# ZongyueQin/SessionSimilaritySearch

Measured on AMD Instinct MI355X. Metric: session queries/sec, higher is better.
Workload: dtype f32

## Files before the change

sessionsimilaritysearch_amd/csrc/ip_topk.hip:

```cpp
#include "scan.h"

namespace sss {

namespace {
constexpr int PROF_RING = 512;
struct Prof {
    bool on = false;
    int n = 0;
    hipEvent_t ev[2 * PROF_RING];
    bool made = false;
};
Prof g_prof[MAX_DEVICES];
}

extern "C" int sss_profile_enable(int on) {
    Prof& p = g_prof[current_device()];
    if (on && !p.made) {
        for (int i = 0; i < 2 * PROF_RING; ++i)
            if (hipEventCreate(&p.ev[i]) != hipSuccess) { set_error("profile_enable: hipEventCreate failed"); return SSS_EHIP; }
        p.made = true;
    }
    p.on = on != 0;
    p.n = 0;
    return SSS_OK;
// ... 12 lines not shown
    *launches = p.n;
    p.n = 0;
    return SSS_OK;
}

static bool fused_shape_ok(int d, int dtype) {
    const int rb = d * elem_bytes(dtype);
    return format_of(dtype) && (rb == 256 || rb == 512 || rb == 1024);
}

int check_scan_source(const char* what, int exact_dtype, int scan_dtype, int d, bool long_rows, const void* c_scan, int corpus_shift,
                      float corpus_resid, long n, long nq) {
    if (long_rows && exact_dtype == DT_I8) {
        set_error("%s: int8 rows (dtype %d) have no long-row scan: d in {256,512,1024} on the fused scan, else the exhaustive kernels", what, DT_I8);
        return SSS_EINVAL;
    }
    if (!(long_rows ? long_shape_ok(d, exact_dtype, scan_dtype) : scan_pair_ok(exact_dtype, scan_dtype, false) && fused_shape_ok(d, scan_dtype))) {
        set_error("%s: no scan of type %d for dtype %d, d %d", what, scan_dtype, exact_dtype, d);
        return SSS_EINVAL;
    }
    if (!c_scan || (reinterpret_cast<uintptr_t>(c_scan) & 15)) {
        set_error("%s: scan image (the %s) missing or not 16-byte aligned", what, format_of(scan_dtype)->name);
        return SSS_EINVAL;
    }
    if (scan_dtype == DT_F16 && (corpus_shift < -160 || corpus_shift > 160 || !(corpus_resid >= 0.f))) {
        set_error("%s: corpus_shift %d outside [-160, 160] or corpus_resid_norm %g not >= 0", what, corpus_shift, (double)corpus_resid);
        return SSS_EINVAL;
    }
    if (n >= (1L << 31) - 1024 || nq >= (1L << 31)) { set_error("%s: n and nq must be < 2^31", what); return SSS_EINVAL; }
    return SSS_OK;
}

ThrArgs thr_args(const void* q, const void* c_exact, int exact_dtype, int scan_dtype, int corpus_shift, float corpus_resid,
                 float corpus_max_norm, const int* qsel, long nsel, long n, int d, int k, int cap, long id_offset) {
    ThrArgs t = {};
    t.Q = q; t.C = c_exact; t.qsel = qsel; t.nsel = (int)nsel; t.d = d; t.dtype = exact_dtype; t.k = k; t.cap = cap; t.n = n;
    t.scan_dtype = scan_dtype; t.corpus_shift = corpus_shift; t.corpus_resid = corpus_resid; t.corpus_max_norm = corpus_max_norm;
    t.id_offset = id_offset;
    return t;
}

extern "C" size_t sss_ip_topk_state_bytes(int64_t nq) { return nq > 0 ? state_words(nq) * 4 : 0; }

extern "C" size_t sss_ip_topk_workspace_bytes(int64_t nq, int64_t n, int d, int k, int dtype) {
    if (nq <= 0 || n <= 0 || k <= 0 || !corpus_dtype_ok(dtype) || !fused_shape_ok(d, dtype)) return 0;
    return make_plan(nq, n, d, k, dtype).total_bytes;
}

static size_t ip_topk_scan_workspace_bytes(long nq, long n, int d, int k, int scan_dtype) {
    if (nq <= 0 || n <= 0 || k <= 0 || !fused_shape_ok(d, scan_dtype)) return 0;
    return make_plan(nq, n, d, k, scan_dtype).total_bytes;
}

extern "C" size_t sss_ip_topk_f16_workspace_bytes(int64_t nq, int64_t n, int d, int k) {
    return ip_topk_scan_workspace_bytes(nq, n, d, k, DT_F16);
}

extern "C" int sss_f16_shift(float amax) { return f16_shift(amax); }

static int ip_topk_impl(const char* what, const void* q, long nq, const void* c_scan, int scan_dtype, int corpus_shift,
                        float corpus_resid, const void* c_exact,
                        int exact_dtype, long n, int d, int k, long id_offset, float corpus_max_norm, float* D_out, long* I_out,
                        int* status, int* unproven_count, void* state, size_t state_bytes, void* ws, size_t ws_bytes,
                        hipStream_t st, const float* bias = nullptr, int d_row = 0) {
    const bool l2 = bias != nullptr;
    if (nq <= 0 || n <= 0 || k <= 0) { set_error("%s: nq, n, k must be positive", what); return SSS_EINVAL; }
    int rc = check_scan_source(what, exact_dtype, scan_dtype, d, false, c_scan, corpus_shift, corpus_resid, n, nq);
    if (rc) return rc;
    if (k > 500) { set_error("%s: k too large (max 500)", what); return SSS_EINVAL; }
    if ((reinterpret_cast<uintptr_t>(ws) & 255) || (reinterpret_cast<uintptr_t>(state) & 15)) {
        set_error("%s: workspace must be 256-byte aligned, state 16-byte aligned", what);
        return SSS_EINVAL;
    }
    if (!state || state_bytes < sss_ip_topk_state_bytes(nq)) { set_error("%s: state %zu < %zu bytes", what, state_bytes, sss_ip_topk_state_bytes(nq)); return SSS_EWORKSPACE; }
    const ScanPlan p = make_plan(nq, n, d, k, scan_dtype);
    if (ws_bytes < p.total_bytes) { set_error("%s: workspace %zu < %zu", what, ws_bytes, p.total_bytes); return SSS_EWORKSPACE; }
    char* w = reinterpret_cast<char*>(ws);

    ScanArgs a;
    a.Q = q; a.C = c_scan; a.nq = (int)nq; a.n = (int)n;
    a.tiles_per_split = p.tiles_per_split; a.total_tiles = p.total_tiles;
    a.S = p.S; a.G = p.G; a.J = p.J; a.Ju = p.Ju; a.cert = p.cert; a.boot = p.boot; a.append = p.append; a.cap = p.cap;
    a.tau_skip = p.tau_skip;
    unsigned* sw = reinterpret_cast<unsigned*>(state);
    a.slots = sw;
    a.cnt = sw + state_off_cnt(nq);
    a.maxlast = reinterpret_cast<unsigned long long*>(sw + state_off_maxlast(nq));
    a.cand = reinterpret_cast<unsigned long long*>(w);
    a.bias = bias; a.corpus_shift = corpus_shift;
    Prof& pr = g_prof[current_device()];
    const bool prof = pr.on && pr.n < PROF_RING;
    if (prof) (void)hipEventRecord(pr.ev[2 * pr.n], st);
    rc = launch_scan(scan_dtype, d, p.tile_rows, a, st);
    if (prof) { (void)hipEventRecord(pr.ev[2 * pr.n + 1], st); ++pr.n; }
    if (rc) return rc;

    SelectArgs s;
    s.Q = q; s.C = c_exact; s.nq = (int)nq; s.d = d; s.dtype = exact_dtype; s.scan_dtype = scan_dtype; s.corpus_shift = corpus_shift; s.corpus_resid = corpus_resid;
    s.k = k; s.K2 = p.K2; s.J = p.J; s.cap = p.cap; s.tau_skip = p.tau_skip;
    s.cand = a.cand; s.slots = a.slots; s.cnt = a.cnt; s.maxlast = a.maxlast;
    s.id_offset = id_offset; s.corpus_max_norm = corpus_max_norm;
    s.D_out = D_out; s.I_out = I_out; s.status = status; s.unproven_count = unproven_count;
    s.metric = l2 ? 1 : 0;
    s.d_row = d_row;
    rc = launch_select(s, st);
    if (rc) (void)hipMemsetAsync(state, 0, sss_ip_topk_state_bytes(nq), st);
    return rc;
}

template <class Prepare, class Select>
static int run_threshold_form(const ThrArgs& t, const void* c_scan, const ScanPlan& p, Prepare prepare, Select select, hipStream_t st,
                              const float* bias = nullptr) {
    int rc = prepare();
    if (rc) return rc;
    ScanArgs a = {};
    a.Q = t.Q; a.C = c_scan; a.nq = t.nsel; a.n = (int)t.n;
    a.tiles_per_split = p.tiles_per_split; a.total_tiles = p.total_tiles;
    a.S = p.S; a.G = p.G; a.J = 0; a.Ju = 0; a.cert = 1; a.boot = 0; a.append = 0; a.cap = p.cap;
    a.slots = nullptr; a.cnt = t.cnt; a.maxlast = nullptr;
    a.cand = const_cast<unsigned long long*>(t.cand);
    a.qsel = t.qsel; a.thr = t.thr;
    a.bias = bias; a.corpus_shift = t.corpus_shift;
    rc = launch_scan(t.scan_dtype, t.d, p.tile_rows, a, st);
    if (rc) return rc;
    return select();
}

constexpr int THR_CAP = 8192;
static size_t thr_head_bytes(long nsel) { return ((size_t)nsel * 8 + 255) & ~(size_t)255; }

extern "C" size_t sss_ip_topk_threshold_workspace_bytes(int64_t nsel, int64_t n, int d, int scan) {
    if (nsel <= 0 || n <= 0 || !fused_shape_ok(d, scan)) return 0;
    return thr_head_bytes(nsel) + make_thr_plan(nsel, n, d, scan, THR_CAP).total_bytes;
}

static int topk_threshold_impl(const char* what, const void* q, const int* qsel, long nsel, const void* c_exact, int exact_dtype,
                               const void* c_scan, int scan_dtype, int corpus_shift, float corpus_resid, long n, int d, int k,
                               long id_offset, float corpus_max_norm, float* D_out, long* I_out, int* status, void* ws, size_t ws_bytes,
                               hipStream_t st, const float* bias = nullptr, int d_row = 0) {
    if (nsel <= 0 || n <= 0 || k <= 0 || !qsel) { set_error("%s: nsel, n, k must be positive", what); return SSS_EINVAL; }
    const int rc = check_scan_source(what, exact_dtype, scan_dtype, d, false, c_scan, corpus_shift, corpus_resid, n, nsel);
    if (rc) return rc;
    if (k > THR_CAP) { set_error("%s: k too large (max %d)", what, THR_CAP); return SSS_EINVAL; }
    if (reinterpret_cast<uintptr_t>(ws) & 255) { set_error("%s: workspace must be 256-byte aligned", what); return SSS_EINVAL; }
    const ScanPlan p = make_thr_plan(nsel, n, d, scan_dtype, THR_CAP);
    if (ws_bytes < thr_head_bytes(nsel) + p.total_bytes) { set_error("%s: workspace %zu < %zu", what, ws_bytes, thr_head_bytes(nsel) + p.total_bytes); return SSS_EWORKSPACE; }
    char* w = reinterpret_cast<char*>(ws);
    ThrArgs t = thr_args(q, c_exact, exact_dtype, scan_dtype, corpus_shift, corpus_resid, corpus_max_norm, qsel, nsel, n, d, k, p.cap,
                         id_offset);
    t.thr = reinterpret_cast<float*>(w);
    t.cnt = reinterpret_cast<unsigned*>(w + (size_t)nsel * 4);
    t.cand = reinterpret_cast<unsigned long long*>(w + thr_head_bytes(nsel));
    t.D_out = D_out; t.I_out = I_out; t.status = status;
    t.metric = bias != nullptr ? 1 : 0;
    t.d_row = d_row;
    return run_threshold_form(t, c_scan, p, [&] { return launch_thr_prepare(t, st); }, [&] { return launch_select_all(t, st); }, st, bias);
}

extern "C" int sss_ip_topk_threshold(const void* q, const int32_t* qsel, int64_t nsel, const void* corpus, int dtype,
                                     const void* scan_image, int scan, int corpus_shift, float corpus_resid_norm, int64_t n, int d,
                                     int k, int64_t id_offset, float corpus_max_norm, float* D_out, int64_t* I_out, int32_t* status,
                                     void* workspace, size_t workspace_bytes, void* stream) {
    hipStream_t st = static_cast<hipStream_t>(stream);
    return topk_threshold_impl("ip_topk_threshold", q, qsel, nsel, corpus, dtype, scan_image, scan, corpus_shift, corpus_resid_norm, n, d,
                               k, id_offset, corpus_max_norm, D_out, I_out, status, workspace, workspace_bytes, st);
}
// ... 185 lines not shown
```

sessionsimilaritysearch_amd/csrc/scan.h:

```cpp
#pragma once
#include "elem.h"

namespace sss {

__host__ __device__ inline int f16_shift(float amax) {
    if (!(amax > 0.f) || !(amax <= 3.4028234663852886e38f)) return 0;
    int e;
    (void)frexpf(amax, &e);
    return 13 - e;
}

constexpr int KP = 16;
constexpr int WG_QUERIES = 256;
constexpr int MAX_SLOTS = 128;
constexpr int SLOT_STRIDE = MAX_SLOTS;
constexpr unsigned ORD_NEG_INF = 0x007FFFFFu;
constexpr double ULP32_REL = 2.4e-7;
constexpr double ULP32_MIN = 1e-44;

static inline int pow2_at_least(int x) { int p = 64; while (p < x) p <<= 1; return p; }

static inline bool long_shape_ok(int d, int exact_dtype, int scan_dtype) {
    return d > 0 && d % 64 == 0 && d * elem_bytes(exact_dtype) <= 16384 && scan_pair_ok(exact_dtype, scan_dtype, true);
}

__device__ __forceinline__ double l2_chain_step(double acc, double q, double c) {
    const double dl = __dsub_rn(q, c);
    return __dadd_rn(acc, __dmul_rn(dl, dl));
}

static inline size_t state_off_cnt(long nq) { return (size_t)nq * MAX_SLOTS; }
static inline size_t state_off_maxlast(long nq) { return (state_off_cnt(nq) + (size_t)nq + 1) & ~(size_t)1; }
static inline size_t state_words(long nq) { return state_off_maxlast(nq) + 2 * (size_t)nq; }

struct ScanPlan {
    int G, S, L, K2, J, Ju, cert, boot, append, tile_rows;
    int tau_skip;
    int total_tiles, tiles_per_split, cap;
    size_t total_bytes;
};

ScanPlan make_plan(long nq, long n, int d, int k, int dtype);

struct ScanArgs {
    const void* Q;
    const void* C;
    int nq, n, tiles_per_split, total_tiles, S, G, J, Ju, cert, boot, append, cap;
    int tau_skip = 0;
    unsigned* slots;
    unsigned* cnt;
    unsigned long long* maxlast;
    unsigned long long* cand;
    const int* qsel = nullptr;
    const float* thr = nullptr;
    const float* bias = nullptr;
    int corpus_shift = 0;
};

ScanPlan make_thr_plan(long nsel, long n, int d, int scan_dtype, int cap);
int launch_scan(int dtype, int d, int tile_rows, const ScanArgs& a, hipStream_t st);
int launch_scan_l2(int dtype, int d, int tile_rows, const ScanArgs& a, hipStream_t st);

struct SelectArgs {
    const void* Q;
    const void* C;
    int nq, d, dtype, k, K2, J, cap;
    int tau_skip = 0;
    int scan_dtype;
    int corpus_shift;
    float corpus_resid;
    const unsigned long long* cand;
    unsigned* slots;
    unsigned* cnt;
    unsigned long long* maxlast;
    long id_offset;
    float corpus_max_norm;
    float* D_out;
    long* I_out;
    int* status;
    int* unproven_count;
    int metric = 0;
    int d_row = 0;
};

int launch_select(const SelectArgs& a, hipStream_t st);

struct ThrArgs {
    const void* Q;
    const void* C;
    const int* qsel;
    int nsel, d, dtype, k, cap;
    long n;
    int scan_dtype, corpus_shift;
    float corpus_resid, corpus_max_norm;
    long id_offset;
    float* thr;
    unsigned* cnt;
    const unsigned long long* cand;
    float* D_out;
    long* I_out;
    int* status;
    double* qb = nullptr;
    int qb_ready = 0;
    int keep = 0;
    int metric = 0;
    int d_row = 0;
};
int launch_thr_prepare(const ThrArgs& a, hipStream_t st);
int launch_select_all(const ThrArgs& a, hipStream_t st);
int launch_long_setup(const ThrArgs& a, int* qsel, void* qimg, float* seed, hipStream_t st);
int launch_bound_prepare(const ThrArgs& a, hipStream_t st);
int launch_range_prepare(const ThrArgs& a, const float* radius, int* qsel, hipStream_t st);
int launch_range_select(const ThrArgs& a, const float* radius, long* counts, int* status, hipStream_t st);
int launch_range_fill(const unsigned* cnt, const unsigned long long* cand, int cap, long nq, const long* lims, long id_offset, float* D,
                      long* I, hipStream_t st);

int check_scan_source(const char* what, int exact_dtype, int scan_dtype, int d, bool long_rows, const void* c_scan, int corpus_shift,
                      float corpus_resid, long n, long nq);
ThrArgs thr_args(const void* q, const void* c_exact, int exact_dtype, int scan_dtype, int corpus_shift, float corpus_resid,
                 float corpus_max_norm, const int* qsel, long nsel, long n, int d, int k, int cap, long id_offset);

size_t topk_of_scores_bytes(long nsel, long n);
int topk_of_scores(const float* scores, const int* qsel, long nsel, long n, int k, long id_offset, int metric, float* D_out,
                   long* I_out, void* tail, hipStream_t st);

}
```

sessionsimilaritysearch_amd/csrc/scan.hip:

```cpp
#include "scan_kernel.h"

namespace sss {

__device__ unsigned g_boot_expired;

extern "C" int sss_scan_boot_expired(int reset) {
    unsigned v = 0, zero = 0;
    if (hipMemcpyFromSymbol(&v, HIP_SYMBOL(g_boot_expired), sizeof(v)) != hipSuccess) { set_error("scan_boot_expired: read failed"); return SSS_EHIP; }
    if (reset && hipMemcpyToSymbol(HIP_SYMBOL(g_boot_expired), &zero, sizeof(zero)) != hipSuccess) { set_error("scan_boot_expired: reset failed"); return SSS_EHIP; }
    return (int)(v > 0x7fffffffu ? 0x7fffffffu : v);
}

int current_device() {
    int dev = 0;
    (void)hipGetDevice(&dev);
    return dev < 0 || dev >= MAX_DEVICES ? 0 : dev;
}

static int pick_splits(long n, int G, int tr) {
    int S = (256 / G) & ~7;
    if (S < 8) S = 8;
    while (S > 8 && (long)S * tr > n) S -= 8;
    return S;
}

constexpr int TR256_MIN_TILES = 24;

static size_t align256(size_t v) { return (v + 255) & ~(size_t)255; }

static ScanPlan make_plan_for(long nq, long n, int d, int k, int dtype, bool want_append);

static bool append_form_fits() {
    static int cached[MAX_DEVICES] = {};
    const int dev = current_device();
    if (cached[dev] == 0) {
        constexpr int lds = 2 * 128 * 256 + 8 * 2048;
        const void* fn = reinterpret_cast<const void*>(&k_scan<256, 128, DT_F16, 8, false, true>);
        int blocks = 0, cus = 0;
        bool ok = hipFuncSetAttribute(fn, hipFuncAttributeMaxDynamicSharedMemorySize, lds) == hipSuccess &&
                  hipOccupancyMaxActiveBlocksPerMultiprocessor(&blocks, fn, 512, lds) == hipSuccess &&
                  hipDeviceGetAttribute(&cus, hipDeviceAttributeMultiprocessorCount, dev) == hipSuccess;
        (void)hipGetLastError();
        cached[dev] = (ok && blocks >= 2 && cus >= 256) ? 1 : 2;
    }
    return cached[dev] == 1;
}

ScanPlan make_plan(long nq, long n, int d, int k, int dtype) {
    const int rb = d * elem_bytes(dtype);
    if (rb == 256 && dtype != DT_F32 && k <= KP && append_form_fits()) {
        const ScanPlan a = make_plan_for(nq, n, d, k, dtype, true);
        if (a.append) return a;
    }
    return make_plan_for(nq, n, d, k, dtype, false);
}
static ScanPlan make_plan_for(long nq, long n, int d, int k, int dtype, bool want_append) {
    ScanPlan p;
    const int rb = d * elem_bytes(dtype);
    const int wgq = rb == 1024 ? 128 : WG_QUERIES;
    p.G = (int)((nq + wgq - 1) / wgq);
    int tr = rb <= 512 ? 128 : 64;
    int S = pick_splits(n, p.G, tr);
    if (rb == 512 && (n + (long)S * 128 - 1) / ((long)S * 128) < 48) { tr = 64; S = pick_splits(n, p.G, tr); }
    if (rb == 256 && dtype != DT_F32 && n / ((long)S * 256) >= TR256_MIN_TILES) tr = 256;
    if (want_append) {
        tr = 128;
        S = pick_splits(n, p.G, tr);
        if ((long)S * p.G > 256 || (long)2 * S * tr * 7 > n) want_append = false;
        else S *= 2;
        if (!want_append) { ScanPlan none; none.append = 0; return none; }
    }
    p.tile_rows = tr;
    p.S = S;
    p.L = 2 * S;
    p.K2 = k + 2 <= KP ? (k + 2 < 8 ? 8 : k + 2) : k <= KP ? KP : k + 12;
    if ((long)p.L * KP < p.K2) p.K2 = p.L * KP;
    p.total_tiles = (int)((n + tr - 1) / tr);
    p.tiles_per_split = (p.total_tiles + S - 1) / S;
    p.cap = p.L * KP;
    const int active_splits = (p.total_tiles + p.tiles_per_split - 1) / p.tiles_per_split;
    p.J = p.K2 <= 128 ? 16 : 64;
    p.cert = 1;
    while (p.J * p.cert < p.K2 && p.cert < KP) p.cert *= 2;
    p.Ju = p.J;
    p.tau_skip = (p.cert == 1 && p.J == 16) ? 16 - p.K2 : 0;
    bool classes_ok = 2 * active_splits >= p.Ju;
    if (p.cert == 1 && p.J == 16 && active_splits < 16) {
        const int zero0 = active_splits < 8 ? 8 - active_splits : 0, zero1 = active_splits < 8 ? 8 : 16 - active_splits;
        classes_ok = zero0 <= (p.tau_skip >> 1) + (p.tau_skip & 1) && zero1 <= (p.tau_skip >> 1);
    }
    if (p.J * p.cert < p.K2 || !classes_ok) { p.J = 0; p.Ju = 0; p.tau_skip = 0; }
    p.boot = (p.J > 0 && p.cert == 1) ? 1 : 0;
    p.append = (want_append && p.boot) ? 1 : 0;
    if (want_append && !p.append) return p;
    if (p.append) p.cap = 2048;
    p.total_bytes = align256((size_t)nq * p.cap * 8);
    return p;
}

ScanPlan make_thr_plan(long nsel, long n, int d, int scan_dtype, int cap) {
    ScanPlan p = {};
    const int rb = d * elem_bytes(scan_dtype);
    const int wgq = rb == 1024 ? 128 : WG_QUERIES;
    p.G = (int)((nsel + wgq - 1) / wgq);
    p.tile_rows = rb <= 512 ? 128 : 64;
    p.S = pick_splits(n, p.G, p.tile_rows);
    p.L = 2 * p.S;
    p.total_tiles = (int)((n + p.tile_rows - 1) / p.tile_rows);
    p.tiles_per_split = (p.total_tiles + p.S - 1) / p.S;
    p.cap = cap;
    p.total_bytes = align256((size_t)nsel * cap * 8);
    return p;
}

int launch_scan(int dtype, int d, int tile_rows, const ScanArgs& a, hipStream_t st) {
    const int rb = d * elem_bytes(dtype);
    if (a.bias != nullptr) return launch_scan_l2(dtype, d, tile_rows, a, st);
    int rc = 1;
    with_dtype<true>(dtype, [&](auto dt) {
        constexpr int DT = decltype(dt)::value;
        rc = launch_shape<DT, 0>(rb, tile_rows, a, st);
    });
    if (rc != 1) return rc;
    set_error("scan: unsupported row size %d bytes", rb);
    return SSS_EINVAL;
}

}
```

sessionsimilaritysearch_amd/csrc/scan_kernel.h:

```cpp
#pragma once
#include "scan.h"
#include "scan_dev.h"

#ifndef SSS_STAGGER
#define SSS_STAGGER 1
#endif
#ifndef SSS_F32_SCHED
#define SSS_F32_SCHED 7
#endif

namespace sss {

extern __device__ unsigned g_boot_expired;

template <int RB, int TR, int DT, int NW, bool THR = false, bool AP = false, int MET = 0>
__global__ __launch_bounds__(NW * 64, AP ? 2 * (NW / 4) : NW / 4) void k_scan(const ScanArgs A) {
    constexpr int H = TR / 64;
    constexpr int CH = RB / 16;
    constexpr int NU = RB / 32;
    constexpr int TILE_BYTES = TR * RB;
    constexpr int LOADS_PER_WAVE = TR * CH / 64 / NW;
    constexpr int WGQ = NW * 32;
    constexpr bool PRECOMP = RB <= 512 && !AP;
    constexpr int TAU_LDS = 2 * TILE_BYTES;
    constexpr bool F32S = (SSS_F32_SCHED & 1) && DT == DT_F32 && !AP && !THR && RB == 512;
    static_assert(CH <= 64, "row longer than one LDS-DMA instruction");
    static_assert(LOADS_PER_WAVE >= 1, "a tile is at least one DMA piece per wave");
    extern __shared__ __attribute__((aligned(16))) char smem[];

    const int nq = A.nq, n = A.n, S = A.S, G = A.G, J = A.J;
    const char* __restrict__ Qb = reinterpret_cast<const char*>(A.Q);
    const char* __restrict__ Cb = reinterpret_cast<const char*>(A.C);
    const int tid = threadIdx.x;
    const int lane = tid & 63;
    const int wave = __builtin_amdgcn_readfirstlane(tid >> 6);
    const int r = lane & 31, h = lane >> 5;

    const int bid = blockIdx.x;
    const int xcd = bid & 7, slot = bid >> 3;
    const int split = xcd * (S >> 3) + slot / G;
    const int g = slot % G;

    const int q_local = wave * 32 + r;
    const int q_glob = g * WGQ + q_local;
    int q_ld = q_glob < nq ? q_glob : nq - 1;
    if constexpr (THR) q_ld = A.qsel[q_ld];
    f32x4 qc[NU];

    float ls[KP];
    int li[KP];
#pragma unroll
    for (int i = 0; i < KP; ++i) { ls[i] = -INFINITY; li[i] = -1; }
    float pend_s = -INFINITY;
    int pend_i = -1;
    constexpr int E = 4;
    float es[E];
    int ei[E];
    int ecnt = 0;
#pragma unroll
    for (int i = 0; i < E; ++i) { es[i] = -INFINITY; ei[i] = -1; }
    float tau = -INFINITY, thr = -INFINITY;
    if constexpr (THR) thr = q_glob < nq ? A.thr[q_glob] : INFINITY;
    float rmax = -INFINITY;
    float pub = -INFINITY;

    int tile_lo = split * A.tiles_per_split;
    int tile_hi = tile_lo + A.tiles_per_split;
    if (tile_hi > A.total_tiles) tile_hi = A.total_tiles;
    const int ntiles = tile_lo < tile_hi ? tile_hi - tile_lo : 0;
    const bool use_tau = !THR && J > 0;
    const bool boot = use_tau && A.boot && ntiles > 0;
    const int nb = boot ? 1 : 0;
    const int niter = ntiles + nb;
    auto tile_of = [&](int i) { return i < ntiles ? tile_lo + i : tile_lo; };
    const int skip = A.tau_skip;

    bool slots_seen = false;
    const unsigned* my_half = nullptr;
    unsigned cls_live = 0;
#ifdef SSS_EXP_NOPAIR
    const bool pair_pub = false;
#else
    const bool pair_pub = A.cert == 1;
#endif
    if (use_tau) {
        cls_live = pair_pub ? (unsigned)(split + (split >> 4)) & 15u : (unsigned)(2 * split + h) % (unsigned)A.Ju;
        my_half = A.slots + (size_t)q_ld * SLOT_STRIDE + h * (J >> 1);
    }
    auto tau_ord = [&]() -> unsigned {
        if (J == 16 && skip > 0) {
            unsigned v[8];
            load8_sc1(my_half, v);
            return tau_select16(v, skip, h);
        }
        unsigned m = 0xFFFFFFFFu;
        for (int v = 0; v < (J >> 1); v += 8) m = min(m, min8_sc1(my_half + v));
        return min(m, (unsigned)__shfl_xor((int)m, 32));
    };
    const unsigned tau_lds = (unsigned)(unsigned long)(lptr_c)smem + TAU_LDS + wave * 2048;
    auto tau_fetch = [&]() {
        int ln = lane;
        asm volatile("" : "+v"(ln));
#pragma unroll
        for (int j = 0; j < 2; ++j) {
            int qi = g * WGQ + wave * 32 + 16 * j + (ln >> 2);
            if (qi > nq - 1) qi = nq - 1;
            const unsigned off = (unsigned)qi * (unsigned)(SLOT_STRIDE * 4) + (unsigned)(ln & 3) * 16u;
            const unsigned dst = __builtin_amdgcn_readfirstlane(tau_lds + j * 1024);
            asm volatile("s_mov_b32 m0, %1\n\ts_nop 0\n\tglobal_load_lds_dwordx4 %0, %2 sc1"
                         : : "v"(off), "s"(dst), "s"(A.slots) : "memory");
        }
    };
    auto tau_read = [&]() -> unsigned {
        const u32x4* p = reinterpret_cast<const u32x4*>(smem + TAU_LDS + wave * 2048 + r * 64 + h * 32);
        const u32x4 a = p[0], b = p[1];
        if (skip > 0) {
            unsigned v[8] = {a.x, a.y, a.z, a.w, b.x, b.y, b.z, b.w};
            return tau_select16(v, skip, h);
        }
        const unsigned m = min(min(min(a.x, a.y), min(a.z, a.w)), min(min(b.x, b.y), min(b.z, b.w)));
        return min(m, (unsigned)__shfl_xor((int)m, 32));
    };
    auto set_tau = [&](unsigned m) {
        if (m > ORD_NEG_INF) tau = fmaxf(tau, ord2f(m - 1));
        thr = AP ? tau : fmaxf(ls[KP - 1], tau);
    };
    auto publish = [&](unsigned cls) {
        float val = rmax;
        bool ok = true;
        if (A.cert > 1) {
            float v2 = ls[1], v4 = ls[3], v8 = ls[7], v16 = ls[KP - 1];
            int i2 = li[1], i4 = li[3], i8 = li[7], i16 = li[KP - 1];
            asm volatile("" : "+v"(v2), "+v"(v4), "+v"(v8), "+v"(v16), "+v"(i2), "+v"(i4), "+v"(i8), "+v"(i16));
            const int c = A.cert;
            val = c == 2 ? v2 : c == 4 ? v4 : c == 8 ? v8 : v16;
            ok = (c == 2 ? i2 : c == 4 ? i4 : c == 8 ? i8 : i16) >= 0;
        }
        if (pair_pub) { val = fmaxf(val, __shfl_xor(val, 32)); ok = h == 0; }
        unsigned cur = 0u;
        if (J == 16 && slots_seen) cur = *reinterpret_cast<const unsigned*>(smem + TAU_LDS + wave * 2048 + r * 64 + cls * 4u);
        if (ok && val > pub && val > tau && f2ord(val) > cur && q_glob < nq) {
            int qq = THR ? q_ld : q_glob;
            asm volatile("" : "+v"(qq));
            __hip_atomic_fetch_max(A.slots + ((size_t)(unsigned)qq * (unsigned)SLOT_STRIDE + cls), f2ord(val), __ATOMIC_RELAXED, __HIP_MEMORY_SCOPE_AGENT);
            pub = val;
        }
    };

    const unsigned lds_base = (unsigned)(unsigned long)(lptr_c)smem;
    auto slot_row = [&](int i) { return ((wave * LOADS_PER_WAVE + i) * 64 + lane) / CH; };
    auto slot_off = [&](int i) {
        const int p = (wave * LOADS_PER_WAVE + i) * 64 + lane;
        const int tr = p / CH, sc = p % CH;
        return (unsigned)(tr * RB + ((sc ^ (tr & 15)) * 16));
    };
    unsigned lane_off[PRECOMP ? LOADS_PER_WAVE : 1];
    if (PRECOMP) {
#pragma unroll
        for (int i = 0; i < LOADS_PER_WAVE; ++i) lane_off[i] = slot_off(i);
    }
    auto stage_piece = [&](int buf, int tile_idx, int i) {
        const long row0 = (long)tile_idx * TR;
        const bool inside = row0 + TR <= (long)n;
        const char* tile_src = Cb + (size_t)row0 * RB;
        const unsigned dst = __builtin_amdgcn_readfirstlane(
            lds_base + buf * TILE_BYTES + (wave * LOADS_PER_WAVE + i) * 1024);
        unsigned off = PRECOMP ? lane_off[PRECOMP ? i : 0] : slot_off(i);
        if (!inside) {
            const int lr = slot_row(i);
            long grow = row0 + lr;
            if (grow > (long)n - 1) grow = (long)n - 1;
            off = (unsigned)((grow - row0) * RB) + (off - (unsigned)(lr * RB));
        }
        asm volatile("s_mov_b32 m0, %1\n\ts_nop 0\n\tglobal_load_lds_dwordx4 %0, %2"
                     : : "v"(off), "s"(dst), "s"(tile_src) : "memory");
    };
    auto stage = [&](int buf, int tile_idx) {
#pragma unroll
        for (int i = 0; i < LOADS_PER_WAVE; ++i) stage_piece(buf, tile_idx, i);
    };

    const int x = h ^ (r & 15);
    f32x16 acc0 = {0}, acc1 = {0};
    [[maybe_unused]] float bcur[MET ? 2 * H : 1];
    [[maybe_unused]] float bscale = 1.f;
    [[maybe_unused]] auto bias_fetch = [&](int tile_idx) {
#pragma unroll
        for (int s = 0; s < 2 * H; ++s) {
            long row = (long)tile_idx * TR + s * 32 + r;
            if (row > (long)n - 1) row = (long)n - 1;
            bcur[s] = h == 0 ? A.bias[row] : 0.f;
        }
    };
    [[maybe_unused]] auto bias_land = [&]() {
#pragma unroll
        for (int s = 0; s < 2 * H; ++s) asm volatile("" : "+v"(bcur[s]));
    };

    auto mfma_sub = [&](int buf, int sub, int next_tile) {
        const char* tile = smem + buf * TILE_BYTES + sub * (64 * RB);
        if constexpr (H == 1) { if (next_tile >= 0) stage(buf ^ 1, next_tile); }
        auto lda = [&](int u) -> const f32x4* {
            const int c = (2 * u) ^ x;
            return reinterpret_cast<const f32x4*>(tile + (r * CH + c) * 16);
        };
        constexpr int PF = DT == DT_F32 ? 1 : AP ? 1 : (RB == 256 ? NU : RB == 512 ? 4 : 2);
        f32x4 as0[NU], as1[NU];
#pragma unroll
        for (int u = 0; u < PF && u < NU; ++u) { const f32x4* p = lda(u); as0[u] = p[0]; as1[u] = p[32 * CH]; }
        const f32x16 zero = {0};
        if constexpr (MET) {
            float b0 = bcur[0], b1 = bcur[1];
#pragma unroll
            for (int s = 1; s < H; ++s) { b0 = sub == s ? bcur[2 * s] : b0; b1 = sub == s ? bcur[2 * s + 1] : b1; }
            acc0 = __builtin_amdgcn_mfma_f32_32x32x2f32(b0, bscale, zero, 0, 0, 0);
            acc1 = __builtin_amdgcn_mfma_f32_32x32x2f32(b1, bscale, zero, 0, 0, 0);
        } else {
            acc0 = zero; acc1 = zero;
        }
        [[maybe_unused]] i32x16 ia0 = {0}, ia1 = {0};
#pragma unroll
        for (int u = 0; u < NU; ++u) {
            if (u + PF < NU) { const f32x4* p = lda(u + PF); as0[u + PF] = p[0]; as1[u + PF] = p[32 * CH]; }
            const f32x4 a0 = as0[u], a1 = as1[u];
            __builtin_amdgcn_sched_barrier(0);
            if constexpr (DT == DT_F32) {
                acc0 = __builtin_amdgcn_mfma_f32_32x32x2f32(a0.x, qc[u].x, acc0, 0, 0, 0);
                acc1 = __builtin_amdgcn_mfma_f32_32x32x2f32(a1.x, qc[u].x, acc1, 0, 0, 0);
                acc0 = __builtin_amdgcn_mfma_f32_32x32x2f32(a0.y, qc[u].y, acc0, 0, 0, 0);
                acc1 = __builtin_amdgcn_mfma_f32_32x32x2f32(a1.y, qc[u].y, acc1, 0, 0, 0);
                acc0 = __builtin_amdgcn_mfma_f32_32x32x2f32(a0.z, qc[u].z, acc0, 0, 0, 0);
                acc1 = __builtin_amdgcn_mfma_f32_32x32x2f32(a1.z, qc[u].z, acc1, 0, 0, 0);
                acc0 = __builtin_amdgcn_mfma_f32_32x32x2f32(a0.w, qc[u].w, acc0, 0, 0, 0);
                acc1 = __builtin_amdgcn_mfma_f32_32x32x2f32(a1.w, qc[u].w, acc1, 0, 0, 0);
            } else if constexpr (DT == DT_BF16) {
                const bf16x8 qb = __builtin_bit_cast(bf16x8, qc[u]);
                acc0 = __builtin_amdgcn_mfma_f32_32x32x16_bf16(__builtin_bit_cast(bf16x8, a0), qb, acc0, 0, 0, 0);
                acc1 = __builtin_amdgcn_mfma_f32_32x32x16_bf16(__builtin_bit_cast(bf16x8, a1), qb, acc1, 0, 0, 0);
            } else if constexpr (DT == DT_F16 || DT == DT_H16) {
                const f16x8 qb = __builtin_bit_cast(f16x8, qc[u]);
                acc0 = __builtin_amdgcn_mfma_f32_32x32x16_f16(__builtin_bit_cast(f16x8, a0), qb, acc0, 0, 0, 0);
                acc1 = __builtin_amdgcn_mfma_f32_32x32x16_f16(__builtin_bit_cast(f16x8, a1), qb, acc1, 0, 0, 0);
            } else if constexpr (DT == DT_I8) {
                const i32x4 qb = __builtin_bit_cast(i32x4, qc[u]);
                ia0 = __builtin_amdgcn_mfma_i32_32x32x32_i8(__builtin_bit_cast(i32x4, a0), qb, ia0, 0, 0, 0);
                ia1 = __builtin_amdgcn_mfma_i32_32x32x32_i8(__builtin_bit_cast(i32x4, a1), qb, ia1, 0, 0, 0);
            } else {
                const bf16x8 A0 = __builtin_bit_cast(bf16x8, a0), A1 = __builtin_bit_cast(bf16x8, a1);
                const bf16x8 qh = __builtin_bit_cast(bf16x8, qc[u < NU / 2 ? u : u - NU / 2]);
                acc0 = __builtin_amdgcn_mfma_f32_32x32x16_bf16(A0, qh, acc0, 0, 0, 0);
                acc1 = __builtin_amdgcn_mfma_f32_32x32x16_bf16(A1, qh, acc1, 0, 0, 0);
                if (u < NU / 2) {
                    const bf16x8 ql = __builtin_bit_cast(bf16x8, qc[u + NU / 2]);
                    acc0 = __builtin_amdgcn_mfma_f32_32x32x16_bf16(A0, ql, acc0, 0, 0, 0);
                    acc1 = __builtin_amdgcn_mfma_f32_32x32x16_bf16(A1, ql, acc1, 0, 0, 0);
                }
            }
            __builtin_amdgcn_sched_barrier(0);
        }
        if constexpr (DT == DT_I8) {
            acc0 = __builtin_convertvector(ia0, f32x16);
            acc1 = __builtin_convertvector(ia1, f32x16);
        }
        if constexpr (H > 1) { if (sub == 0 && next_tile >= 0) stage(buf ^ 1, next_tile); }
    };

    auto block_max = [&](const f32x16& a, float& q0, float& q1, float& q2, float& q3) {
        q0 = fmaxf(fmaxf(a[0], a[1]), fmaxf(a[2], a[3]));
        q1 = fmaxf(fmaxf(a[4], a[5]), fmaxf(a[6], a[7]));
        q2 = fmaxf(fmaxf(a[8], a[9]), fmaxf(a[10], a[11]));
        q3 = fmaxf(fmaxf(a[12], a[13]), fmaxf(a[14], a[15]));
        return fmaxf(fmaxf(q0, q1), fmaxf(q2, q3));
    };
    auto insert_block = [&](const f32x16& a, int base) {
// ... 10 lines not shown
                    if (__builtin_amdgcn_ballot_w64(pass && pend_i >= 0) != 0) {
                        list_insert<KP>(ls, li, pend_s, pend_i);
                        pend_s = -INFINITY; pend_i = -1;
                        thr = fmaxf(ls[KP - 1], tau);
                    }
                    const bool still = a[j] > thr;
                    pend_s = still ? a[j] : pend_s;
                    pend_i = still ? base + (j & 3) + 8 * (j >> 2) : pend_i;
                }
            }
        };
        walk(q0, 0); walk(q1, 4); walk(q2, 8); walk(q3, 12);
    };
    auto flush = [&](bool need) {
        if (need && q_glob < nq) {
            const unsigned at = atomicAdd(A.cnt + q_glob, (unsigned)ecnt);
            unsigned long long* dst = A.cand + (size_t)q_glob * A.cap;
            unsigned long long lost = 0ull;
#pragma unroll
            for (int i = 0; i < E; ++i) {
                if (i < ecnt) {
                    const unsigned long long key = make_key(es[i], ei[i]);
                    if (at + (unsigned)i < (unsigned)A.cap) dst[at + i] = key;
                    else lost = lost > key ? lost : key;
                }
            }
            if (lost != 0ull && A.maxlast != nullptr) atomicMax(A.maxlast + q_glob, lost);
        }
        ecnt = need ? 0 : ecnt;
    };
    auto append_block = [&](const f32x16& a, int base) {
        float q0, q1, q2, q3;
        const float m = block_max(a, q0, q1, q2, q3);
        if (__builtin_amdgcn_ballot_w64(m > thr) == 0) return;
        auto walk = [&](float qm, int j0) {
            if (__builtin_amdgcn_ballot_w64(qm > thr) == 0) return;
#pragma unroll
            for (int jj = 0; jj < 4; ++jj) {
                const int j = j0 + jj;
                const bool pass = a[j] > thr;
                if (__builtin_amdgcn_ballot_w64(pass) != 0) {
                    const bool full = pass && ecnt == E;
                    if (__builtin_amdgcn_ballot_w64(full) != 0) flush(full);
#pragma unroll
                    for (int i = E - 1; i > 0; --i) { es[i] = pass ? es[i - 1] : es[i]; ei[i] = pass ? ei[i - 1] : ei[i]; }
                    es[0] = pass ? a[j] : es[0];
                    ei[0] = pass ? base + (j & 3) + 8 * (j >> 2) : ei[0];
                    ecnt += pass ? 1 : 0;
                }
            }
        };
        walk(q0, 0); walk(q1, 4); walk(q2, 8); walk(q3, 12);
    };
    auto emit_block = [&](const f32x16& a, int base) {
        float q0, q1, q2, q3;
        const float m = block_max(a, q0, q1, q2, q3);
        if (__builtin_amdgcn_ballot_w64(m > thr) == 0) return;
#pragma unroll
        for (int j = 0; j < 16; ++j) {
            if (a[j] > thr) {
                const unsigned pos = atomicAdd(A.cnt + q_glob, 1u);
                if (pos < (unsigned)A.cap) A.cand[(size_t)q_glob * A.cap + pos] = make_key(a[j], base + (j & 3) + 8 * (j >> 2));
            }
        }
    };
    const bool two_ahead = H > 1 && niter > 1;
    if (ntiles > 0) stage(0, tile_lo);
    if (two_ahead) stage(1, tile_of(1));
    if constexpr (MET) {
        int q_shift = 0;
        load_queries<RB, DT>(Qb, q_ld, h, qc, &q_shift);
        if constexpr (DT == DT_F16) {
            const int e = A.corpus_shift + q_shift;
            bscale = ldexpf(1.f, e < -126 ? -126 : e > 127 ? 127 : e);
        }
        bias_fetch(tile_of(0));
    } else {
        load_queries<RB, DT>(Qb, q_ld, h, qc);
    }
    asm volatile("s_waitcnt vmcnt(0)" ::: "memory");
    __syncthreads();
    if constexpr (MET) bias_land();

    const int T = niter * H;
    long row0_of_step = 0;
    constexpr bool TAU_EVERY_TILE = TR >= 512;
    auto refresh_at = [&](int i) {
        if (i == 1 && boot && !TAU_EVERY_TILE) return false;
        if (TAU_EVERY_TILE || i <= 4) return true;
        const int sh = 30 - __builtin_clz(i);
        return (i & ((1 << sh) - 1)) == 0;
    };
    auto tile_top = [&](int i) {
        if (!use_tau || i == 0) return;
        if (J == 16) {
            if (!refresh_at(i)) return;
            publish(cls_live);
            tau_fetch();
            return;
        }
        const int ii = i - (wave >= 4 ? 1 : 0);
        if (ii >= 2 && (ii <= 8 || (ii & (ii - 1)) == 0 || (ii & 15) == 0)) set_tau(tau_ord());
        publish(cls_live);
    };
    auto tile_end = [&](int i) {
        const bool pre = boot && i == 0;
        if (pre) publish(cls_live);
        if constexpr (MET) { if (i + 1 < niter) bias_fetch(tile_of(i + 1)); }
        asm volatile("s_waitcnt vmcnt(0)" ::: "memory");
        if (use_tau && J == 16 && i > 0 && refresh_at(i)) { set_tau(tau_read()); slots_seen = true; }
        __syncthreads();
        if (pre) {
            unsigned m = 0;
            for (int it = 0; it < (AP ? 1024 : 24); ++it) {
                m = tau_ord();
                if (__builtin_amdgcn_ballot_w64(m == 0) == 0) break;
                __builtin_amdgcn_s_sleep(16);
            }
            if constexpr (!MET) {
                if (lane == 0 && __builtin_amdgcn_ballot_w64(m == 0 && q_glob < nq) != 0) atomicAdd(&g_boot_expired, 1u);
            }
            set_tau(m);
        }
        if constexpr (MET) bias_land();
    };
    auto score_mfma = [&](int t) {
        const int i = (int)((unsigned)t / (unsigned)H), sub = (int)((unsigned)t % (unsigned)H);
        if (sub == 0) tile_top(i);
        const int next_tile = (i + 1 < niter && !(two_ahead && i == 0)) ? tile_of(i + 1) : -1;
        mfma_sub(i & 1, sub, next_tile);
        row0_of_step = (long)tile_of(i) * TR + sub * 64;
        if (row0_of_step + 64 > n) {
#pragma unroll
            for (int j = 0; j < 16; ++j) {
                const int rr = (int)row0_of_step + 4 * h + (j & 3) + 8 * (j >> 2);
                if (rr >= n) acc0[j] = -INFINITY;
                if (rr + 32 >= n) acc1[j] = -INFINITY;
            }
        }
    };
    auto score_tree = [&]() -> float {
        float m0 = vmax3(acc0[0], acc0[1], acc0[2]), m1 = vmax3(acc1[0], acc1[1], acc1[2]);
#pragma unroll
        for (int j = 3; j < 15; j += 2) { m0 = vmax3(m0, acc0[j], acc0[j + 1]); m1 = vmax3(m1, acc1[j], acc1[j + 1]); }
        const float m = vmax3(m0, m1, acc0[15]);
        const float mm = vmax3(m, acc1[15], rmax);
        rmax = mm;
        return vmax3(m, acc1[15], acc1[15]);
    };
    const int t_live = nb * H;
    const bool defer = SSS_STAGGER && NW == 8 && (DT == DT_SPLIT || DT == DT_BF16 || DT == DT_H16 || DT == DT_I8) && wave >= 4;
    int t = 0;
    if constexpr (AP || THR) {
        t = T;
        for (int i = 0; i < niter; ++i) {
            tile_top(i);
            const int tile = tile_of(i);
            const int next_tile = (i + 1 < niter && !(two_ahead && i == 0)) ? tile_of(i + 1) : -1;
            const int row_base = tile * TR;
            const bool ragged = row_base + TR > n;
            const bool live = i >= nb;
            if constexpr (THR) {
                if (g * WGQ + wave * 32 >= nq) {
                    if (next_tile >= 0) stage((i & 1) ^ 1, next_tile);
                    tile_end(i);
                    continue;
                }
            }
#pragma unroll
            for (int sub = 0; sub < H; ++sub) {
                mfma_sub(i & 1, sub, next_tile);
                const int row0 = row_base + sub * 64;
                if (ragged) {
#pragma unroll
                    for (int j = 0; j < 16; ++j) {
                        const int rr = row0 + 4 * h + (j & 3) + 8 * (j >> 2);
                        if (rr >= n) acc0[j] = -INFINITY;
                        if (rr + 32 >= n) acc1[j] = -INFINITY;
                    }
                }
                const float m = score_tree();
                if (live && __builtin_amdgcn_ballot_w64(m > thr) != 0) {
                    append_block(acc0, row0 + 4 * h);
                    append_block(acc1, row0 + 32 + 4 * h);
                }
            }
            tile_end(i);
        }
    }
    if constexpr (F32S) {
        constexpr bool SPREAD = (SSS_F32_SCHED & 2) != 0, EARLY_TREE = (SSS_F32_SCHED & 4) != 0;
        static_assert(LOADS_PER_WAVE + 1 < NU, "a DMA piece per k-group, behind k-groups 1 .. LOADS_PER_WAVE");
        const unsigned frag_lane = (unsigned)(r * CH) * 16u;
        f32x4 nf0 = {0}, nf1 = {0};
        auto frag_ptr = [&](unsigned step_off, int u) -> const f32x4* {
            const int c = (2 * u) ^ x;
            return reinterpret_cast<const f32x4*>(smem + step_off + frag_lane + c * 16);
        };
        auto read_first = [&](unsigned step_off) { const f32x4* p = frag_ptr(step_off, 0); nf0 = p[0]; nf1 = p[32 * CH]; };
        float tm0 = -INFINITY;
        auto step = [&](int t) -> float {
            const int i = (int)((unsigned)t / (unsigned)H), sub = (int)((unsigned)t % (unsigned)H);
            const unsigned off = (unsigned)((i & 1) * TILE_BYTES + sub * (64 * RB));
            f32x4 as0[NU], as1[NU];
            as0[0] = nf0; as1[0] = nf1;
            const f32x16 zero = {0};
            if constexpr (MET) {
                float b0 = bcur[0], b1 = bcur[1];
#pragma unroll
                for (int s = 1; s < H; ++s) { b0 = sub == s ? bcur[2 * s] : b0; b1 = sub == s ? bcur[2 * s + 1] : b1; }
                acc0 = __builtin_amdgcn_mfma_f32_32x32x2f32(b0, bscale, zero, 0, 0, 0);
                acc1 = __builtin_amdgcn_mfma_f32_32x32x2f32(b1, bscale, zero, 0, 0, 0);
            } else {
                acc0 = zero; acc1 = zero;
            }
            auto fetch = [&](int u) { const f32x4* p = frag_ptr(off, u); as0[u] = p[0]; as1[u] = p[32 * CH]; };
            auto mfma8 = [&](int u) {
                const f32x4 a0 = as0[u], a1 = as1[u];
                __builtin_amdgcn_sched_barrier(0);
                acc0 = __builtin_amdgcn_mfma_f32_32x32x2f32(a0.x, qc[u].x, acc0, 0, 0, 0);
                acc1 = __builtin_amdgcn_mfma_f32_32x32x2f32(a1.x, qc[u].x, acc1, 0, 0, 0);
                acc0 = __builtin_amdgcn_mfma_f32_32x32x2f32(a0.y, qc[u].y, acc0, 0, 0, 0);
                acc1 = __builtin_amdgcn_mfma_f32_32x32x2f32(a1.y, qc[u].y, acc1, 0, 0, 0);
                acc0 = __builtin_amdgcn_mfma_f32_32x32x2f32(a0.z, qc[u].z, acc0, 0, 0, 0);
                acc1 = __builtin_amdgcn_mfma_f32_32x32x2f32(a1.z, qc[u].z, acc1, 0, 0, 0);
                acc0 = __builtin_amdgcn_mfma_f32_32x32x2f32(a0.w, qc[u].w, acc0, 0, 0, 0);
                acc1 = __builtin_amdgcn_mfma_f32_32x32x2f32(a1.w, qc[u].w, acc1, 0, 0, 0);
                __builtin_amdgcn_sched_barrier(0);
            };
            fetch(1);
            mfma8(0);
            if (sub == 0) tile_top(i);
            const int next_tile = (sub == 0 && i + 1 < niter && !(two_ahead && i == 0)) ? tile_of(i + 1) : -1;
            const long nrow0 = (long)next_tile * TR;
            const bool dma_plain = next_tile >= 0 && nrow0 + TR <= (long)n;
            const char* dma_src = Cb + (size_t)nrow0 * RB;
            const unsigned dma_dst = __builtin_amdgcn_readfirstlane(lds_base + ((i & 1) ^ 1) * TILE_BYTES + wave * LOADS_PER_WAVE * 1024);
            row0_of_step = (long)tile_of(i) * TR + sub * 64;
            const bool ragged_step = row0_of_step + 64 > n;
            const bool ends_tile = sub == H - 1 && !(boot && i == 0);
            if (next_tile >= 0 && (!dma_plain || !SPREAD)) stage((i & 1) ^ 1, next_tile);
#pragma unroll
            for (int u = 1; u < NU - 1; ++u) {
                fetch(u + 1);
                mfma8(u);
                if constexpr (SPREAD) {
                    if (u <= LOADS_PER_WAVE && dma_plain)
                        asm volatile("s_mov_b32 m0, %1\n\ts_nop 0\n\tglobal_load_lds_dwordx4 %0, %2"
                                     : : "v"(lane_off[u - 1]), "s"(dma_dst + (u - 1) * 1024), "s"(dma_src) : "memory");
                }
            }
            constexpr int u = NU - 1;
            if (ends_tile) {
                asm volatile("" : "+v"(as0[u]), "+v"(as1[u]));
                tile_end(i);
            }
            if (t + 1 < T && (sub < H - 1 || ends_tile))
                read_first(sub == H - 1 ? (unsigned)(((i + 1) & 1) * TILE_BYTES) : off + 64 * RB);
            if constexpr (!EARLY_TREE) {
                mfma8(u);
            } else {
                const f32x4 a0 = as0[u], a1 = as1[u];
                __builtin_amdgcn_sched_barrier(0);
                acc0 = __builtin_amdgcn_mfma_f32_32x32x2f32(a0.x, qc[u].x, acc0, 0, 0, 0);
                acc0 = __builtin_amdgcn_mfma_f32_32x32x2f32(a0.y, qc[u].y, acc0, 0, 0, 0);
                acc0 = __builtin_amdgcn_mfma_f32_32x32x2f32(a0.z, qc[u].z, acc0, 0, 0, 0);
                acc0 = __builtin_amdgcn_mfma_f32_32x32x2f32(a0.w, qc[u].w, acc0, 0, 0, 0);
                __builtin_amdgcn_sched_barrier(0);
                acc1 = __builtin_amdgcn_mfma_f32_32x32x2f32(a1.x, qc[u].x, acc1, 0, 0, 0);
                acc1 = __builtin_amdgcn_mfma_f32_32x32x2f32(a1.y, qc[u].y, acc1, 0, 0, 0);
                __builtin_amdgcn_sched_barrier(0);
                if (ragged_step) {
#pragma unroll
                    for (int j = 0; j < 16; ++j)
                        if ((int)row0_of_step + 4 * h + (j & 3) + 8 * (j >> 2) >= n) acc0[j] = -INFINITY;
                }
                tm0 = vmax3(acc0[0], acc0[1], acc0[2]);
#pragma unroll
                for (int j = 3; j < 15; j += 2) tm0 = vmax3(tm0, acc0[j], acc0[j + 1]);
                __builtin_amdgcn_sched_barrier(0);
                acc1 = __builtin_amdgcn_mfma_f32_32x32x2f32(a1.z, qc[u].z, acc1, 0, 0, 0);
                acc1 = __builtin_amdgcn_mfma_f32_32x32x2f32(a1.w, qc[u].w, acc1, 0, 0, 0);
                __builtin_amdgcn_sched_barrier(0);
            }
            if (ragged_step) {
#pragma unroll
                for (int j = 0; j < 16; ++j) {
                    const int rr = (int)row0_of_step + 4 * h + (j & 3) + 8 * (j >> 2);
                    if (!EARLY_TREE && rr >= n) acc0[j] = -INFINITY;
                    if (rr + 32 >= n) acc1[j] = -INFINITY;
                }
            }
            if constexpr (!EARLY_TREE) return score_tree();
            float m1 = vmax3_settled(acc1[0], acc1[1], acc1[2]);
#pragma unroll
            for (int j = 3; j < 15; j += 2) m1 = vmax3(m1, acc1[j], acc1[j + 1]);
            const float m = vmax3(tm0, m1, acc0[15]);
            rmax = vmax3(m, acc1[15], rmax);
            return vmax3(m, acc1[15], acc1[15]);
        };
        if (T > 0) read_first(0);
        while (t < T) {
            bool rare = false;
            for (; t < T; ++t) {
                const float m = step(t);
                if (t < t_live) {
                    if (t == t_live - 1) {
                        tile_end(0);
                        if (t + 1 < T) read_first((unsigned)TILE_BYTES);
                    }
                    continue;
                }
                if (__builtin_amdgcn_ballot_w64(m > thr) != 0) { rare = true; break; }
            }
            if (!rare) break;
            insert_block(acc0, (int)row0_of_step + 4 * h);
            insert_block(acc1, (int)row0_of_step + 32 + 4 * h);
            ++t;
        }
    }
    while (!F32S && t < T) {
        bool rare = false;
        for (; t < T; ++t) {
            const bool last = (unsigned)t % (unsigned)H == H - 1;
            const bool early = defer && t >= t_live;
            score_mfma(t);
            if (early && last) tile_end((int)((unsigned)t / (unsigned)H));
            const float m = score_tree();
            if (t >= t_live && __builtin_amdgcn_ballot_w64(m > thr) != 0) { rare = true; break; }
            if (!early && last) tile_end((int)((unsigned)t / (unsigned)H));
        }
        if (!rare) break;
        if constexpr (THR) {
            emit_block(acc0, (int)row0_of_step + 4 * h);
            emit_block(acc1, (int)row0_of_step + 32 + 4 * h);
        } else if constexpr (AP) {
            append_block(acc0, (int)row0_of_step + 4 * h);
            append_block(acc1, (int)row0_of_step + 32 + 4 * h);
        } else {
            insert_block(acc0, (int)row0_of_step + 4 * h);
            insert_block(acc1, (int)row0_of_step + 32 + 4 * h);
        }
        if (!defer && (unsigned)t % (unsigned)H == H - 1) tile_end((int)((unsigned)t / (unsigned)H));
        ++t;
    }
    if constexpr (THR) { flush(ecnt > 0); return; }
    if constexpr (AP) flush(ecnt > 0);
    list_insert<KP>(ls, li, pend_s, pend_i);
    if (!AP && q_glob < nq) {
        int nreal = 0;
#pragma unroll
        for (int i = 0; i < KP; ++i) nreal += li[i] >= 0 ? 1 : 0;
        if (nreal > 0) {
            const unsigned base = atomicAdd(A.cnt + q_glob, (unsigned)nreal);
            unsigned long long* dst = A.cand + (size_t)q_glob * A.cap + base;
#pragma unroll
            for (int i = 0; i < KP; ++i)
                if (i < nreal) dst[i] = make_key(ls[i], li[i]);
            if (nreal == KP) atomicMax(A.maxlast + q_glob, (unsigned long long)make_key(ls[KP - 1], li[KP - 1]));
        }
    }
}

template <int RB, int TR, int DT, int NW, int MET, bool THR, bool AP = false>
static int launch_form(const ScanArgs& a, hipStream_t st) {
    const size_t lds = 2 * (size_t)TR * RB + NW * 2048;
    const int rc = opt_in_lds(reinterpret_cast<const void*>(&k_scan<RB, TR, DT, NW, THR, AP, MET>), "k_scan", lds);
    if (rc) return rc;
    hipLaunchKernelGGL((k_scan<RB, TR, DT, NW, THR, AP, MET>), dim3(a.S * a.G), dim3(NW * 64), lds, st, a);
    return check_launch("k_scan");
}
template <int RB, int TR, int DT, int NW, int MET>
static int launch_one(const ScanArgs& a, hipStream_t st) {
    if (a.thr != nullptr) {
        if constexpr (TR == (RB <= 512 ? 128 : 64)) return launch_form<RB, TR, DT, NW, MET, true>(a, st);
        set_error("scan: threshold form not built for %d-row tiles of %d-byte rows", TR, RB);
        return SSS_EINVAL;
    }
    if (a.append) {
        if constexpr (RB == 256 && TR == 128 && DT != DT_F32) return launch_form<RB, TR, DT, NW, MET, false, true>(a, st);
        set_error("scan: append form not built for this shape");
        return SSS_EINVAL;
    }
    return launch_form<RB, TR, DT, NW, MET, false>(a, st);
}
template <int DT, int MET>
static int launch_shape(int rb, int tile_rows, const ScanArgs& a, hipStream_t st) {
    if (rb == 256) return tile_rows == 256 ? launch_one<256, 256, DT, 8, MET>(a, st) : launch_one<256, 128, DT, 8, MET>(a, st);
    if (rb == 512) return tile_rows == 128 ? launch_one<512, 128, DT, 8, MET>(a, st) : launch_one<512, 64, DT, 8, MET>(a, st);
    if (rb == 1024) return launch_one<1024, 64, DT, 4, MET>(a, st);
    return 1;
}

}
```

Measured before the change: 500,200.

## Balance f32 scan splits at 64-row step granularity instead of whole tiles

Adds an even-split rule that divides the corpus into 64-row steps and hands each split an equal count, replacing whole-tile splits for the 512-row-byte f32 scan path. The kernel offsets the corpus and bias pointers per split, handles partial final tiles, and shortens the bootstrap phase to a single step when the new sched bit is set. The aim is to cut load imbalance and tail waste across workgroups, at the cost of more complex tile-end logic and possible edge cases with ragged tiles and candidate row offsets.

```diff
diff --git a/sessionsimilaritysearch_amd/csrc/ip_topk.hip b/sessionsimilaritysearch_amd/csrc/ip_topk.hip
--- a/sessionsimilaritysearch_amd/csrc/ip_topk.hip
+++ b/sessionsimilaritysearch_amd/csrc/ip_topk.hip
@@ -118,6 +118,7 @@
     a.tiles_per_split = p.tiles_per_split; a.total_tiles = p.total_tiles;
     a.S = p.S; a.G = p.G; a.J = p.J; a.Ju = p.Ju; a.cert = p.cert; a.boot = p.boot; a.append = p.append; a.cap = p.cap;
     a.tau_skip = p.tau_skip;
+    a.step_q = p.step_q; a.step_rem = p.step_rem;
     unsigned* sw = reinterpret_cast<unsigned*>(state);
     a.slots = sw;
     a.cnt = sw + state_off_cnt(nq);
diff --git a/sessionsimilaritysearch_amd/csrc/scan.h b/sessionsimilaritysearch_amd/csrc/scan.h
--- a/sessionsimilaritysearch_amd/csrc/scan.h
+++ b/sessionsimilaritysearch_amd/csrc/scan.h
@@ -1,5 +1,6 @@
 #pragma once
 #include "elem.h"
+#include "split_rule.h"
 
 namespace sss {
 
@@ -38,6 +39,7 @@
     int tau_skip;
     int total_tiles, tiles_per_split, cap;
     size_t total_bytes;
+    int step_q = 0, step_rem = 0;
 };
 
 ScanPlan make_plan(long nq, long n, int d, int k, int dtype);
@@ -55,6 +57,7 @@
     const float* thr = nullptr;
     const float* bias = nullptr;
     int corpus_shift = 0;
+    int step_q = 0, step_rem = 0;
 };
 
 ScanPlan make_thr_plan(long nsel, long n, int d, int scan_dtype, int cap);
diff --git a/sessionsimilaritysearch_amd/csrc/scan.hip b/sessionsimilaritysearch_amd/csrc/scan.hip
--- a/sessionsimilaritysearch_amd/csrc/scan.hip
+++ b/sessionsimilaritysearch_amd/csrc/scan.hip
@@ -78,7 +78,13 @@
     p.total_tiles = (int)((n + tr - 1) / tr);
     p.tiles_per_split = (p.total_tiles + S - 1) / S;
     p.cap = p.L * KP;
-    const int active_splits = (p.total_tiles + p.tiles_per_split - 1) / p.tiles_per_split;
+    int active_splits = (p.total_tiles + p.tiles_per_split - 1) / p.tiles_per_split;
+    if (rb == 512 && dtype == DT_F32 && (SSS_F32_SCHED & 9) == 9) {
+        const EvenSplits e = even_splits(n, S);
+        p.step_q = e.q;
+        p.step_rem = e.rem;
+        active_splits = even_active_splits(e, S);
+    }
     p.J = p.K2 <= 128 ? 16 : 64;
     p.cert = 1;
     while (p.J * p.cert < p.K2 && p.cert < KP) p.cert *= 2;
diff --git a/sessionsimilaritysearch_amd/csrc/scan_kernel.h b/sessionsimilaritysearch_amd/csrc/scan_kernel.h
--- a/sessionsimilaritysearch_amd/csrc/scan_kernel.h
+++ b/sessionsimilaritysearch_amd/csrc/scan_kernel.h
@@ -6,7 +6,7 @@
 #define SSS_STAGGER 1
 #endif
 #ifndef SSS_F32_SCHED
-#define SSS_F32_SCHED 7
+#define SSS_F32_SCHED 31
 #endif
 
 namespace sss {
@@ -28,7 +28,8 @@
     static_assert(LOADS_PER_WAVE >= 1, "a tile is at least one DMA piece per wave");
     extern __shared__ __attribute__((aligned(16))) char smem[];
 
-    const int nq = A.nq, n = A.n, S = A.S, G = A.G, J = A.J;
+    const int nq = A.nq, S = A.S, G = A.G, J = A.J;
+    int n = A.n;
     const char* __restrict__ Qb = reinterpret_cast<const char*>(A.Q);
     const char* __restrict__ Cb = reinterpret_cast<const char*>(A.C);
     const int tid = threadIdx.x;
@@ -67,11 +68,34 @@
     int tile_lo = split * A.tiles_per_split;
     int tile_hi = tile_lo + A.tiles_per_split;
     if (tile_hi > A.total_tiles) tile_hi = A.total_tiles;
-    const int ntiles = tile_lo < tile_hi ? tile_hi - tile_lo : 0;
+    int ntiles_split = tile_lo < tile_hi ? tile_hi - tile_lo : 0;
+    int row_off_split = 0, nst_split = 0;
+    if constexpr (F32S) {
+        row_off_split = tile_lo * TR;
+        nst_split = ntiles_split * H;
+        if ((A.step_q | A.step_rem) != 0) {
+            EvenSplits e;
+            e.q = A.step_q; e.rem = A.step_rem;
+            long lo, hi;
+            even_split_rows(e, n, split, &lo, &hi);
+            row_off_split = (int)lo;
+            nst_split = (int)((hi - lo + 63) >> 6);
+            ntiles_split = (nst_split + H - 1) / H;
+        }
+        tile_lo = 0;
+        n -= row_off_split;
+        Cb += (size_t)(unsigned)row_off_split * RB;
+    }
+    const int ntiles = ntiles_split;
+    [[maybe_unused]] const int row_off = F32S ? row_off_split : 0, nst = F32S ? nst_split : 0;
+    [[maybe_unused]] const float* bias_rows = nullptr;
+    if constexpr (MET) bias_rows = A.bias + row_off;
     const bool use_tau = !THR && J > 0;
     const bool boot = use_tau && A.boot && ntiles > 0;
     const int nb = boot ? 1 : 0;
     const int niter = ntiles + nb;
+    constexpr int NBS = (SSS_F32_SCHED & 16) ? 1 : H;
+    [[maybe_unused]] const int nbs = !boot ? 0 : NBS < nst ? NBS : nst;
     auto tile_of = [&](int i) { return i < ntiles ? tile_lo + i : tile_lo; };
     const int skip = A.tau_skip;
 
@@ -189,7 +213,7 @@
         for (int s = 0; s < 2 * H; ++s) {
             long row = (long)tile_idx * TR + s * 32 + r;
             if (row > (long)n - 1) row = (long)n - 1;
-            bcur[s] = h == 0 ? A.bias[row] : 0.f;
+            bcur[s] = h == 0 ? bias_rows[row] : 0.f;
         }
     };
     [[maybe_unused]] auto bias_land = [&]() {
@@ -366,7 +390,7 @@
     __syncthreads();
     if constexpr (MET) bias_land();
 
-    const int T = niter * H;
+    const int T = F32S ? nst + nbs : niter * H;
     long row0_of_step = 0;
     constexpr bool TAU_EVERY_TILE = TR >= 512;
     auto refresh_at = [&](int i) {
@@ -387,10 +411,10 @@
         if (ii >= 2 && (ii <= 8 || (ii & (ii - 1)) == 0 || (ii & 15) == 0)) set_tau(tau_ord());
         publish(cls_live);
     };
-    auto tile_end = [&](int i) {
-        const bool pre = boot && i == 0;
+    auto tile_end = [&](int i, int pre_sel = -1, bool tile_done = true) {
+        const bool pre = pre_sel < 0 ? boot && i == 0 : pre_sel != 0;
         if (pre) publish(cls_live);
-        if constexpr (MET) { if (i + 1 < niter) bias_fetch(tile_of(i + 1)); }
+        if constexpr (MET) { if (tile_done && i + 1 < niter) bias_fetch(tile_of(i + 1)); }
         asm volatile("s_waitcnt vmcnt(0)" ::: "memory");
         if (use_tau && J == 16 && i > 0 && refresh_at(i)) { set_tau(tau_read()); slots_seen = true; }
         __syncthreads();
@@ -432,7 +456,7 @@
         rmax = mm;
         return vmax3(m, acc1[15], acc1[15]);
     };
-    const int t_live = nb * H;
+    const int t_live = F32S ? nbs : nb * H;
     const bool defer = SSS_STAGGER && NW == 8 && (DT == DT_SPLIT || DT == DT_BF16 || DT == DT_H16 || DT == DT_I8) && wave >= 4;
     int t = 0;
     if constexpr (AP || THR) {
@@ -484,7 +508,9 @@
         auto read_first = [&](unsigned step_off) { const f32x4* p = frag_ptr(step_off, 0); nf0 = p[0]; nf1 = p[32 * CH]; };
         float tm0 = -INFINITY;
         auto step = [&](int t) -> float {
-            const int i = (int)((unsigned)t / (unsigned)H), sub = (int)((unsigned)t % (unsigned)H);
+            const bool closing = t >= nst;
+            const int i = closing ? ntiles : (int)((unsigned)t / (unsigned)H), sub = closing ? t - nst : (int)((unsigned)t % (unsigned)H);
+            const bool tile_last = sub == H - 1 || t == nst - 1 || t == T - 1;
             const unsigned off = (unsigned)((i & 1) * TILE_BYTES + sub * (64 * RB));
             f32x4 as0[NU], as1[NU];
             as0[0] = nf0; as1[0] = nf1;
@@ -522,7 +548,7 @@
             const unsigned dma_dst = __builtin_amdgcn_readfirstlane(lds_base + ((i & 1) ^ 1) * TILE_BYTES + wave * LOADS_PER_WAVE * 1024);
             row0_of_step = (long)tile_of(i) * TR + sub * 64;
             const bool ragged_step = row0_of_step + 64 > n;
-            const bool ends_tile = sub == H - 1 && !(boot && i == 0);
+            const bool ends_tile = tile_last && !(t == nbs - 1);
             if (next_tile >= 0 && (!dma_plain || !SPREAD)) stage((i & 1) ^ 1, next_tile);
 #pragma unroll
             for (int u = 1; u < NU - 1; ++u) {
@@ -537,10 +563,10 @@
             constexpr int u = NU - 1;
             if (ends_tile) {
                 asm volatile("" : "+v"(as0[u]), "+v"(as1[u]));
-                tile_end(i);
-            }
-            if (t + 1 < T && (sub < H - 1 || ends_tile))
-                read_first(sub == H - 1 ? (unsigned)(((i + 1) & 1) * TILE_BYTES) : off + 64 * RB);
+                tile_end(i, 0);
+            }
+            if (t + 1 < T && (!tile_last || ends_tile))
+                read_first(tile_last ? (unsigned)(((i + 1) & 1) * TILE_BYTES) : off + 64 * RB);
             if constexpr (!EARLY_TREE) {
                 mfma8(u);
             } else {
@@ -590,16 +616,17 @@
                 const float m = step(t);
                 if (t < t_live) {
                     if (t == t_live - 1) {
-                        tile_end(0);
-                        if (t + 1 < T) read_first((unsigned)TILE_BYTES);
+                        const bool tile_done = (unsigned)t % (unsigned)H == H - 1 || t == nst - 1;
+                        tile_end(0, 1, tile_done);
+                        if (t + 1 < T && tile_done) read_first((unsigned)TILE_BYTES);
                     }
                     continue;
                 }
                 if (__builtin_amdgcn_ballot_w64(m > thr) != 0) { rare = true; break; }
             }
             if (!rare) break;
-            insert_block(acc0, (int)row0_of_step + 4 * h);
-            insert_block(acc1, (int)row0_of_step + 32 + 4 * h);
+            insert_block(acc0, (int)row0_of_step + row_off + 4 * h);
+            insert_block(acc1, (int)row0_of_step + row_off + 32 + 4 * h);
             ++t;
         }
     }
diff --git a/sessionsimilaritysearch_amd/csrc/split_rule.h b/sessionsimilaritysearch_amd/csrc/split_rule.h
--- /dev/null
+++ b/sessionsimilaritysearch_amd/csrc/split_rule.h
@@ -0,0 +1,37 @@
+#pragma once
+
+#if defined(__HIPCC__) || defined(__CUDACC__)
+#define SSS_SPLIT_HD __host__ __device__
+#else
+#define SSS_SPLIT_HD
+#endif
+
+namespace sss {
+
+constexpr int SPLIT_STEP_ROWS = 64;
+
+struct EvenSplits {
+    int q, rem;
+};
+
+SSS_SPLIT_HD inline EvenSplits even_splits(long n, int S) {
+    const long steps = (n + SPLIT_STEP_ROWS - 1) / SPLIT_STEP_ROWS;
+    EvenSplits e;
+    e.q = (int)(steps / S);
+    e.rem = (int)(steps % S);
+    return e;
+}
+
+SSS_SPLIT_HD inline void even_split_rows(EvenSplits e, long n, int s, long* lo, long* hi) {
+    const long first = (long)s * e.q + (s < e.rem ? s : e.rem);
+    const long count = e.q + (s < e.rem ? 1 : 0);
+    long a = first * SPLIT_STEP_ROWS, b = (first + count) * SPLIT_STEP_ROWS;
+    if (b > n) b = n;
+    if (count == 0) a = b = n;
+    *lo = a;
+    *hi = b;
+}
+
+SSS_SPLIT_HD inline int even_active_splits(EvenSplits e, int S) { return e.q > 0 ? S : e.rem; }
+
+}
```

After: 500,400, median of 2. Within noise of the previous version (+0.0%).
